# dhruvmetha/rapid-locomotion-rl

Hardware: AMD Instinct MI355X
Metric: env-steps/sec, 4096 Mini Cheetah envs, 1/2/4/8 MI355X; PPO iters/sec (higher is better)
Workload: dtype f32; 1 GPU; 4096 Mini Cheetah envs flat terrain (4096 per GPU), PPO teacher policy (BASELINE configs[1]); envs_per_gpu=4096, global_envs=4096, global_batch_env_steps_per_iter=98304, parallelism=dp1, world_size=1, policy=ActorCritic 42/18/630->12, random init; teacher PPO + student adaptation update

## Files before the change

### include/lrl.h

```cpp
#ifndef LRL_H_
#define LRL_H_

#include <stddef.h>
#include <stdint.h>

#ifdef __cplusplus
extern "C" {
#endif

#define LRL_ABI_VERSION 6

#define LRL_OK 0
#define LRL_E_INVALID (-1)
#define LRL_E_HIP (-2)
#define LRL_E_NOMEM (-3)
#define LRL_E_NOGPU (-4)

#define LRL_MAX_BODIES 20
#define LRL_MAX_SPHERES 40
#define LRL_NUM_DOF 12
#define LRL_NUM_LEGS 4
#define LRL_MAX_OBS 256
#define LRL_MAX_HEIGHT_POINTS 192
#define LRL_MAX_REWARD_TERMS 24
// ... 516 lines not shown
                           int32_t zero, void* stream);

int32_t lrl_curriculum_sample(uint32_t* mt_key, int32_t* mt_pos, const double* weights, int32_t nbins,
                              const double* grid, const double* half, int32_t n, double* cmds, int64_t* bins);
int32_t lrl_curriculum_update_weights(double* weights, const double* axes, int32_t nx, int32_t ny, int32_t nz,
                                      const int64_t* centres, int32_t n, double local_range);
double lrl_np_sum_f64(const double* a, int64_t n);

#ifdef __cplusplus
}
#endif

#include "lrl_vision.h"
#include "lrl_depth_sense.h"
#include "lrl_history_shift.h"

#endif
```

### rapid-locomotion-rl_amd/csrc/lrl_ppo.hip

```cpp
#include <hip/hip_runtime.h>
#include <math.h>
#include <stdint.h>
#include <stdlib.h>
#include <string.h>

#include <algorithm>
#include <initializer_list>
#include <mutex>
#include <vector>

#include "../../include/lrl.h"
#include "../../include/lrl_philox.h"
#include "lrl_gemm.h"
#include "lrl_launch.h"

namespace lrl {

constexpr float LOG_SQRT_2PI = 0.91893853320467274178f;
constexpr int HEAD_ROWS = 32;
constexpr int HEAD_THREADS = 256;
constexpr int HEAD_W = 128;
constexpr int MAX_ACT = 16;
constexpr int HEAD_NA = 12;
constexpr int MAX_LAT = 32;
// ... 272 lines not shown
    }
    P[hp_b4a(NA) + t] = sb;
    P[hp_std(NA) + t] = ss;
  } else if (t == 16) {
    float sb = 0.f;
    for (int r = 0; r < nrows; ++r) sb += DR[r][1];
    P[hp_b4c(NA)] = sb;
  } else if (t >= 32 && t < 35) {
    const int c = t - 32;
    float s = 0.f;
    for (int r = 0; r < nrows; ++r) s += SC[r][c];
    P[hp_kl(NA) + c] = s;
  }
}

struct ActHeadArgs {
  const float* h3;
  const float *w4a, *b4a, *w4c, *b4c, *stdv;
  const float *obs, *priv, *hist, *eps;
  int n, na, no, np;
  uint64_t seed, counter;
  int64_t row_offset;
  float *actions, *mu, *values, *logp;
  lrl_rollout_store store;
  int store_row, do_store;
  float* xa_out;
  float* hist_shift;
  int hist_slot;
};

template <int NT = HEAD_THREADS>
__device__ __forceinline__ void copy_rows(const float* __restrict__ src, int64_t sld, float* __restrict__ dst,
                                          int64_t dld, int nrows, int cols, int t) {
  if (((((uintptr_t)src | (uintptr_t)dst) & 7) == 0) && (((sld | dld | cols) & 1) == 0)) {
    const int c2 = cols / 2, n = nrows * c2;
    for (int i0 = t; i0 < n; i0 += 8 * NT) {
      float2 v[8];
#pragma unroll
      for (int u = 0; u < 8; ++u) {
        const int i = i0 + u * NT, r = i / c2, c = i - r * c2;
        if (i < n) v[u] = reinterpret_cast<const float2*>(src + r * sld)[c];
      }
#pragma unroll
// ... 131 lines not shown
    const float m = MU[r][j], sd = a.stdv[j];
    float act;
    MU[r][j] = act_draw(a.eps, a.row_offset, a.seed, a.counter, g, j, na, m, sd, act);
    a.actions[(int64_t)g * na + j] = act;
    if (a.mu) a.mu[(int64_t)g * na + j] = m;
    if (a.do_store) {
      const int64_t o = (so + g) * na + j;
      a.store.actions[o] = act;
      a.store.mu[o] = m;
      a.store.sigma[o] = sd;
    }
  }
  __syncthreads();
  if (t < nrows) {
    const int g = r0 + t;
    float lp = 0.f;
    for (int j = 0; j < na; ++j) lp += MU[t][j];
    float vs[ACT_Q];
#pragma unroll
    for (int q = 0; q < ACT_Q; ++q) vs[q] = VP[t][q];
#pragma unroll
    for (int w = ACT_Q / 2; w >= 1; w /= 2)
#pragma unroll
      for (int q = 0; q < w; ++q) vs[q] = vs[2 * q] + vs[2 * q + 1];
    const float v = vs[0] + a.b4c[0];
    if (a.values) a.values[g] = v;
    if (a.logp) a.logp[g] = lp;
    if (a.do_store) {
      a.store.values[so + g] = v;
      a.store.logp[so + g] = lp;
// ... 167 lines not shown

struct FusedActArgs {
  const float* w;
  lrl_ppo_net net;
  const float *obs, *priv, *hist, *eps;
  int n, xs;
  uint32_t vec;
  uint64_t seed, counter;
  int64_t row_offset;
  float *actions, *mu, *values, *logp;
  lrl_rollout_store store;
  int store_row, do_store;
  float* xa_out;
  float* hist_shift;
  int hist_slot;
};

template <bool PRESET, int RB>
__device__ __forceinline__ void fa_encoder(const FusedActArgs& a, float* X, float* HE1, float* MID, int r0, int nrows,
                                           unsigned long long& fa_t) {
  constexpr int R = 16 * RB, NT = 256 * RB;
  const lrl_ppo_net& nt = a.net;
  const int t = threadIdx.x;
  const int no = nt.num_obs, np = nt.num_priv, PP = 36, EP2 = nt.enc_h1 + 4;
  for (int e = t; e < R * a.xs; e += NT) {
    const int r = e / a.xs, c = e - r * a.xs;
    X[r * FA_XP + c] = (r < nrows && c < no) ? a.obs[(int64_t)(r0 + r) * no + c] : 0.f;
  }
  for (int e = t; e < R * 32; e += NT) {
    const int r = e >> 5, c = e & 31;
// ... 247 lines not shown
          const int64_t o = (so + g) * NA + j;
          a.store.actions[o] = act;
          a.store.mu[o] = m;
          a.store.sigma[o] = sd;
        }
      }
      __syncthreads();
      if (t < nrows) {
        const int g = r0 + t;
        float lp = 0.f;
        for (int j = 0; j < NA; ++j) lp += MU[t * 16 + j];
        if (a.logp) a.logp[g] = lp;
        if (a.do_store) a.store.logp[so + g] = lp;
      }
    } else {
      for (int e = t; e < HEAD_W; e += OA_THREADS) HW[e] = w[nt.w4c + e];
      __syncthreads();
      for (int e = t; e < OA_R * 16; e += OA_THREADS) {
        const int r = e & (OA_R - 1), q = e / OA_R;
        float s = 0.f;
        for (int k = q * (HEAD_W / 16); k < (q + 1) * (HEAD_W / 16); ++k) s = fmaf(H3[r * OA_H3P + k], HW[k], s);
        VP[r * 16 + q] = s;
      }
      __syncthreads();
      FA_PROF(8)
      if (t < nrows) {
        const int g = r0 + t;
        float vs[16];
#pragma unroll
        for (int q = 0; q < 16; ++q) vs[q] = VP[t * 16 + q];
// ... 740 lines not shown
  if (reset) {
    unsigned long long z[12] = {0};
    if (hipMemcpyToSymbol(HIP_SYMBOL(g_act_prof), z, sizeof(z)) != hipSuccess) return -2;
  }
  return 12;
#else
  (void)out;
  (void)reset;
  return 0;
#endif
}

static int32_t ppo_act(const lrl_ppo_net* net, const float* params, const float* obs, const float* priv,
                       const float* hist, int32_t n, const float* eps, uint64_t seed, uint64_t counter,
                       int64_t row_offset, float* actions, float* mu, float* values, float* logp, const lrl_rollout_store* store,
                       int32_t store_row, void* workspace, void* stream, float* hist_shift, int32_t hist_slot) {
  if (int rc = check_net(net)) return rc;
  if (hist_shift && (hist_shift != hist || !store || !store->hist || hist_slot <= 0 || store->hist_dim % hist_slot != 0))
    return lrl_set_error(LRL_E_INVALID, "lrl_ppo_act_shift: hist_shift must be hist, with a history store and a slot "
                                        "width that divides its hist_dim");
  if (!params || !obs || (!priv && !net->plain) || !actions || !workspace || n <= 0)
    return lrl_set_error(LRL_E_INVALID, "lrl_ppo_act: null argument or n <= 0");
  if (store && (!store->obs || (!store->priv && priv) || !store->actions || !store->values || !store->logp ||
                !store->mu || !store->sigma || store->hist_dim < 0 ||
                (store->hist_ld != 0 && store->hist_ld < store->hist_dim)))
    return lrl_set_error(LRL_E_INVALID, "lrl_ppo_act: incomplete rollout store");
  const lrl_ppo_net& nt = *net;
  hipStream_t st = static_cast<hipStream_t>(stream);
  auto io = [&](auto& a) {
    a.obs = obs; a.priv = priv; a.hist = hist; a.eps = eps; a.n = n;
    a.seed = seed; a.counter = counter; a.row_offset = row_offset;
    a.actions = actions; a.mu = mu; a.values = values; a.logp = logp;
    if (store) a.store = *store;
    a.store_row = store_row; a.do_store = store ? 1 : 0;
    a.hist_shift = hist_shift; a.hist_slot = hist_slot;
  };
  const bool full = !nt.plain;
  if (full && fused_act_fits(nt, n)) {
    static const bool ok = [] {
      auto set = [](const void* f) {
        return hipFuncSetAttribute(f, hipFuncAttributeMaxDynamicSharedMemorySize, OA_LDS_BYTES) == hipSuccess;
      };
      return set(reinterpret_cast<const void*>(act_fused_kernel<true>)) &&
             set(reinterpret_cast<const void*>(act_fused_kernel<false>));
    }();
    if (!ok) return lrl_set_error(LRL_E_HIP, "lrl_ppo_act: fused kernel LDS attribute");
    FusedActArgs fa{};
    fa.w = params; fa.net = nt; fa.xs = xs_of(nt);
    io(fa);
    launch_act_fused(fa, true, st);
// ... 30 lines not shown
extern "C" int32_t lrl_ppo_act(const lrl_ppo_net* net, const float* params, const float* obs, const float* priv,
                               const float* hist, int32_t n, const float* eps, uint64_t seed, uint64_t counter,
                               int64_t row_offset, float* actions, float* mu, float* values, float* logp, const lrl_rollout_store* store,
                               int32_t store_row, void* workspace, void* stream) {
  return ppo_act(net, params, obs, priv, hist, n, eps, seed, counter, row_offset, actions, mu, values, logp, store, store_row,
                 workspace, stream, nullptr, 0);
}

extern "C" int32_t lrl_ppo_act_shift(const lrl_ppo_net* net, const float* params, const float* obs, const float* priv,
                                     const float* hist, int32_t n, const float* eps, uint64_t seed, uint64_t counter,
                                     int64_t row_offset, float* actions, float* mu, float* values, float* logp,
                                     const lrl_rollout_store* store, int32_t store_row, void* workspace, void* stream,
                                     float* hist_shift, int32_t hist_slot) {
  return ppo_act(net, params, obs, priv, hist, n, eps, seed, counter, row_offset, actions, mu, values, logp, store, store_row,
                 workspace, stream, hist_shift, hist_slot);
}

extern "C" int64_t lrl_ppo_act_student_workspace_bytes(const lrl_ppo_net* net, int32_t n) {
  if (check_net(net) || net->plain || n <= 0) return -1;
  return make_student_plan(*net, n, nullptr).bytes;
}

extern "C" int32_t lrl_ppo_act_student(const lrl_ppo_net* net, const float* params, const float* obs,
                                       const float* hist, int32_t hist_ld, int32_t n, float* mean, float* latent,
                                       void* workspace, void* stream) {
  if (int rc = check_net(net)) return rc;
  if (net->plain) return lrl_set_error(LRL_E_INVALID, "lrl_ppo_act_student: a plain net has no adaptation module");
  if (!params || !obs || !hist || !mean || !workspace || n <= 0)
    return lrl_set_error(LRL_E_INVALID, "lrl_ppo_act_student: null argument or n <= 0");
  const lrl_ppo_net& nt = *net;
// ... 11 lines not shown
  body_forward(g, L.body, P);
  g.forward(L.mean, P.h3, nullptr, Buf{mean, nt.num_actions}, false);
  if (g.rc) return lrl_set_error(g.rc, "lrl_ppo_act_student: GEMM launch failed");
  if (latent &&
      hipMemcpy2DAsync(latent, (size_t)nt.latent * 4, lat.p, (size_t)lat.ld * 4, (size_t)nt.latent * 4, n,
                       hipMemcpyDeviceToDevice, st) != hipSuccess)
    return lrl_set_error(LRL_E_HIP, "lrl_ppo_act_student: latent copy failed");
  return hipGetLastError() == hipSuccess ? 0 : lrl_set_error(LRL_E_HIP, "lrl_ppo_act_student: launch failed");
}

extern "C" int64_t lrl_ppo_workspace_bytes(const lrl_ppo_net* net, int32_t batch) {
  if (check_net(net) || batch <= 0) return -1;
  return make_plan(*net, batch, nullptr).bytes;
}

extern "C" int32_t lrl_ppo_forward_backward(const lrl_ppo_net* net, const float* params, float* grads,
                                            const lrl_ppo_batch* bt, const lrl_ppo_hparams* hp, void* workspace,
                                            lrl_ppo_ctrl* ctrl, void* stream) {
  if (int rc = check_net(net)) return rc;
  if (!bt || !hp || !params || !grads || !workspace || !ctrl || bt->batch <= 0)
    return lrl_set_error(LRL_E_INVALID, "lrl_ppo_forward_backward: null argument");
  const lrl_ppo_net& n = *net;
  const int B = bt->batch;
  const bool full = !n.plain;
  Plan P = make_plan(n, B, static_cast<char*>(workspace));
  hipStream_t st = static_cast<hipStream_t>(stream);
  G g{st, params, B, P.part, P.part + P.part_floats};
  g.tanh_act = n.plain;
  const Net net_l = layers_of(n);
  const Layer(&enc)[3] = net_l.enc;
  const Layer(&body)[3] = net_l.body;
  PlaneJob pj[PL_MAIN];
  if (full) {
    main_plane_jobs(n, params, P.wpl, pj);
    if (int rc = split_planes(pj, PL_MAIN, gemm_x6p_enabled(), st))
      return lrl_set_error(rc, "lrl_ppo_forward_backward: planes launch failed");
    g.with(pj);
  }
  const In priv{bt->priv, n.num_priv};
  prep_x(n, bt->obs, bt->rows, B, P.xa, st);
  if (full) encoder_forward(g, enc, priv, bt->rows, P, cols_from(P.xa, n.num_obs));
  body_forward(g, body, P);
  if (g.rc) return lrl_set_error(g.rc, "lrl_ppo_forward_backward: forward GEMM launch failed");
  SegList L{};
  launch_loss_head(n, params, grads, bt, hp, ctrl, P, g.part, L, st);
  g.backward_data(body[2], P.dh3, P.dh2, P.h2);
  g.backward_data(body[1], P.dh2, P.dh1, P.h1);
  if (full) g.backward_data(net_l.dlat, P.dh1, P.dlat, In{});
  enum { DWE3, DHE2, DWE2, DHE1, DWE1, DW3, DW2, DW1, NJOBS };
  GemmJob jobs[NJOBS];
  const int first = full ? 0 : DW3;
  g.collect(jobs, first, NJOBS);
  if (full) {
    g.weight_grad(enc[2], P.dlat, P.he2, nullptr, grads, L);
    g.backward_data(enc[2], P.dlat, P.dhe2, P.he2);
// ... 29 lines not shown
    return lrl_set_error(LRL_E_HIP, "lrl_ppo_forward_backward: stream fork failed");
  for (int s = 0; s < ns && !rc; ++s) {
    const int lead = sets[s].i[0];
    const bool timed = full && sets[s].n == 1 && lead == DW2;
    if (timed) timer_begin(st);
    rc = launch_jobs(jobs, sets[s].i, sets[s].n, fk && lead < DW3 ? fk->st : st);
    if (timed) timer_end(st);
    if (fk && lead == DWE1 && hipEventRecord(fk->done, fk->st) != hipSuccess)
      return lrl_set_error(LRL_E_HIP, "lrl_ppo_forward_backward: stream fork failed");
  }
  if (fk && hipStreamWaitEvent(st, fk->done, 0) != hipSuccess)
    return lrl_set_error(LRL_E_HIP, "lrl_ppo_forward_backward: stream join failed");
  if (rc) return lrl_set_error(rc, "lrl_ppo_forward_backward: backward GEMM launch failed");
  launch_seg(L, st);
  return hipGetLastError() == hipSuccess ? 0 : lrl_set_error(LRL_E_HIP, "lrl_ppo_forward_backward: launch failed");
}

extern "C" int32_t lrl_ppo_optimizer_step(const lrl_ppo_net* net, float* params, const float* grads, float* exp_avg,
                                          float* exp_avg_sq, int64_t step, float grad_scale,
                                          const lrl_ppo_hparams* hp, void* workspace, lrl_ppo_ctrl* ctrl,
                                          void* stream) {
  if (int rc = check_net(net)) return rc;
  if (!params || !grads || !exp_avg || !exp_avg_sq || !hp || !workspace || !ctrl || step < 1)
    return lrl_set_error(LRL_E_INVALID, "lrl_ppo_optimizer_step: bad argument");
  const lrl_ppo_net& n = *net;
  hipStream_t st = static_cast<hipStream_t>(stream);
  double* norm_part = static_cast<double*>(workspace);
  const int64_t len = n.main_end - n.main_begin;
  hipLaunchKernelGGL(sumsq_kernel, dim3(NORM_BLOCKS), dim3(256), 0, st, grads + n.main_begin, len, norm_part);
  const double bc1 = 1.0 - pow((double)hp->beta1, (double)step);
// ... 248 lines not shown
```

### rapid-locomotion-rl_amd/lrl/_abi.py

```python
import ctypes as C
import os
import re

_HERE = os.path.dirname(os.path.abspath(__file__))
LIB_PATH = os.environ.get("LRL_LIB") or os.path.join(os.path.dirname(_HERE), "csrc", "liblrl.so")

MAX_BODIES, MAX_SPHERES, NUM_DOF, NUM_LEGS, MAX_OBS, MAX_REWARD_TERMS, NUM_PRIV = 20, 40, 12, 4, 256, 24, 18
MAX_HEIGHT_POINTS = 192
f32, i32, u32 = C.c_float, C.c_int32, C.c_uint32

REWARD_TERMS = ["lin_vel_z", "ang_vel_xy", "orientation", "base_height", "torques", "energy",
                "energy_expenditure", "dof_vel", "dof_acc", "action_rate", "collision", "survival",
                "dof_pos_limits", "dof_vel_limits", "torque_limits", "tracking_lin_vel", "tracking_ang_vel",
                "feet_air_time", "stumble", "stand_still", "feet_contact_forces"]

STEP_PHYSICS, STEP_HISTORY, STEP_INJECT_UNIFORM = 1, 2, 4

(T_ROOT_STATE, T_DOF_POS, T_DOF_VEL, T_CONTACT_FORCE, T_RIGID_BODY_STATE, T_TORQUES, T_ACTIONS, T_LAST_ACTIONS,
 T_LAST_DOF_VEL, T_LAST_ROOT_VEL, T_COMMANDS, T_OBS, T_PRIV_OBS, T_OBS_HISTORY, T_REWARD, T_RESET, T_TIME_OUT,
 T_EPISODE_LENGTH, T_EPISODE_SUMS, T_COMMAND_SUMS, T_FEET_AIR_TIME, T_LAST_CONTACTS, T_FRICTION, T_RESTITUTION,
 T_PAYLOAD, T_COM_DISPLACEMENT, T_MOTOR_STRENGTH, T_KP_FACTOR, T_KD_FACTOR, T_ENV_ORIGINS, T_BASE_LIN_VEL,
 T_BASE_ANG_VEL, T_PROJECTED_GRAVITY, T_JOINT_POS_TARGET, T_MEASURED_HEIGHTS, T_NUM) = range(36)


# ... 194 lines not shown
    return struct


def _fill_array(arr, v):
    for i, x in enumerate(v):
        if isinstance(arr[i], C.Array):
            _fill_array(arr[i], x)
        else:
            arr[i] = x


_CSRC = os.path.join(os.path.dirname(_HERE), "csrc")
_HEADER = os.path.join(os.path.dirname(os.path.dirname(_HERE)), "include", "lrl.h")
_SENSE_HEADER = os.path.join(os.path.dirname(_HEADER), "lrl_depth_sense.h")
_SHIFT_HEADER = os.path.join(os.path.dirname(_HEADER), "lrl_history_shift.h")


def source_hash():
    import hashlib
    with open(os.path.join(_CSRC, "Makefile")) as f:
        mk = f.read()
    h = hashlib.sha256()
    for var in ("SRCS", "HDRS"):
        for name in re.search(rf"^{var} = (.*)$", mk, re.M).group(1).split():
            with open(os.path.join(_CSRC, name), "rb") as f:
                h.update(f.read())
    return h.hexdigest()[:16]


MIRRORS = {"lrl_model": LrlModel, "lrl_env_params": LrlEnvParams, "lrl_group_params": LrlGroupParams,
# ... 36 lines not shown

_lib = None


def lib():
    global _lib
    if _lib is None:
        if not os.path.exists(LIB_PATH):
            raise RuntimeError(f"liblrl.so not built ({LIB_PATH}); run __graft_entry__.build()")
        L = C.CDLL(LIB_PATH)
        L.lrl_build_hash.restype = C.c_char_p
        built, want = L.lrl_build_hash().decode(), source_hash()
        if built != want and not os.environ.get("LRL_LIB"):
            raise RuntimeError(f"{LIB_PATH} was built from other sources (hash {built}, tree {want}); "
                               "rebuild it: __graft_entry__.build()")
        for header in (_HEADER, _SENSE_HEADER, _SHIFT_HEADER):
            with open(header) as f:
                for name, (restype, argtypes) in signatures(f.read()).items():
                    fn = getattr(L, name)
                    fn.restype, fn.argtypes = restype, argtypes
        _lib = L
    return _lib


def check(rc):
    if rc != 0:
        msg = lib().lrl_last_error()
        raise RuntimeError(f"liblrl error {rc}: {msg.decode() if msg else ''}")
    return rc


# ... 13 lines not shown
```

### rapid-locomotion-rl_amd/lrl/ppo/actor_critic.py

```python
import ctypes as C

import torch

import torch.nn as nn

from .. import _abi
from ..config import ArgsProto


class AC_Args(ArgsProto):
    init_noise_std = 1.0
    actor_hidden_dims = [512, 256, 128]
    critic_hidden_dims = [512, 256, 128]
    activation = "elu"
    adaptation_module_branch_hidden_dims = [[256, 32]]
    env_factor_encoder_branch_input_dims = [18]
    env_factor_encoder_branch_latent_dims = [18]
    env_factor_encoder_branch_hidden_dims = [[256, 128]]


def get_activation(name):
    return {"elu": nn.ELU(), "selu": nn.SELU(), "relu": nn.ReLU(), "crelu": nn.ReLU(), "lrelu": nn.LeakyReLU(),
            "tanh": nn.Tanh(), "sigmoid": nn.Sigmoid()}.get(name)

# ... 147 lines not shown
        net = self.flatten_parameters()
        ws = getattr(self, "_student_ws", None)
        if ws is None or ws[0] != n or ws[1].device != dev:
            nbytes = _abi.lib().lrl_ppo_act_student_workspace_bytes(C.byref(net), n)
            if nbytes < 0:
                raise RuntimeError("lrl_ppo_act_student_workspace_bytes rejected the network")
            ws = self._student_ws = (n, torch.empty(nbytes, dtype=torch.uint8, device=dev))
        mean = torch.empty(n, self.num_actions, device=dev)
        latent = torch.empty(n, net.latent, device=dev)
        _abi.check(_abi.lib().lrl_ppo_act_student(net, self._flat.data_ptr(), obs.data_ptr(), hist.data_ptr(),
                                                  hist.stride(0), n, mean.data_ptr(), latent.data_ptr(),
                                                  ws[1].data_ptr(), _abi.stream_of(dev)))
        return mean, latent

    def act_fused(self, obs, priv, hist=None, eps=None, seed=0, counter=0, store=None, store_row=0, row_offset=0,
                  shift_history=False):
        n = obs.shape[0]
        dev = obs.device
        assert obs.is_contiguous() and (priv is None or priv.is_contiguous()) and obs.dtype == torch.float32
        net = self.flatten_parameters()
        ws = getattr(self, "_act_ws", None)
        if ws is None or ws[0] != n or ws[1].device != dev:
            nbytes = _abi.lib().lrl_ppo_act_workspace_bytes(C.byref(net), n)
            if nbytes < 0:
                raise RuntimeError("lrl_ppo_act_workspace_bytes rejected the network")
            ws = self._act_ws = (n, torch.empty(nbytes, dtype=torch.uint8, device=dev))
        actions = torch.empty(n, self.num_actions, device=dev)
        mu = torch.empty(n, self.num_actions, device=dev)
        values = torch.empty(n, 1, device=dev)
        logp = torch.empty(n, device=dev)
        priv_p, hist_p, eps_p = (t.data_ptr() if t is not None else None for t in (priv, hist, eps))
        if shift_history:
            if hist is None or store is None or not hist.is_contiguous():
                raise ValueError("shift_history needs a contiguous history and a rollout store")
            _abi.check(_abi.lib().lrl_ppo_act_shift(net, self._flat.data_ptr(), obs.data_ptr(), priv_p, hist_p, n, eps_p,
                                                    seed, counter, row_offset, actions.data_ptr(), mu.data_ptr(),
                                                    values.data_ptr(), logp.data_ptr(), store, store_row,
                                                    ws[1].data_ptr(), _abi.stream_of(dev), hist_p, obs.shape[1]))
            return actions, mu, values, logp
        _abi.check(_abi.lib().lrl_ppo_act(net, self._flat.data_ptr(), obs.data_ptr(), priv_p, hist_p, n, eps_p, seed,
                                          counter, row_offset, actions.data_ptr(), mu.data_ptr(), values.data_ptr(),
                                          logp.data_ptr(), store, store_row, ws[1].data_ptr(), _abi.stream_of(dev)))
        return actions, mu, values, logp
```

### rapid-locomotion-rl_amd/lrl/ppo/ppo.py

```python
import ctypes as C
import os

import torch

import torch.distributed as dist
import torch.nn as nn
import torch.nn.functional as F

from .. import _abi
from ..config import ArgsProto
from .actor_critic import ActorCritic
from .rollout_storage import RolloutStorage


_SNAPSHOTS = max(2, int(os.environ.get("LRL_ENC_SNAPSHOTS", "4")))


class PPO_Args(ArgsProto):
    value_loss_coef = 1.0
    use_clipped_value_loss = True
    clip_param = 0.2
    entropy_coef = 0.01
    num_learning_epochs = 5
    num_mini_batches = 4
# ... 41 lines not shown
                                                            lr=self.args.adaptation_module_learning_rate)
        self.transition = RolloutStorage.Transition()
        self._lr = float(self.args.learning_rate)
        self.async_losses = False
        self._lr_dev = None
        self.fused = (torch.device(device).type == "cuda") if fused is None else fused
        self.seed = seed
        self.row_offset = 0
        self._act_counter = 0
        self._store = None
        self.grad_allreduce = _collective()
        self._native = None
        self.record_lr = False
        self.overlap_adaptation = True
        self.lr_trace = []
        if self.fused:
            self.actor_critic.flatten_parameters()

    def init_storage(self, num_envs, num_transitions_per_env, actor_obs_shape, privileged_obs_shape, obs_history_shape,
                     action_shape):
        self.storage = self.storage_class(num_envs, num_transitions_per_env, actor_obs_shape, privileged_obs_shape,
                                          obs_history_shape, action_shape, self.device)
        self._store = self.storage.store_desc() if self.fused else None

    def test_mode(self):
        self.actor_critic.eval()

    def train_mode(self):
        self.actor_critic.train()

    def act(self, obs, privileged_obs, obs_history, eps=None, shift_history=False):
        if shift_history and not (self.fused and obs_history.is_contiguous()):
            raise ValueError("shift_history needs the native act and a contiguous history")
        if self.fused:
            self._act_counter += 1
            a, mu, v, lp = self.actor_critic.act_fused(
                obs.contiguous(), privileged_obs.contiguous(), obs_history.contiguous(), eps=eps, seed=self.seed,
                counter=self._act_counter, store=self._store, store_row=self.storage.step,
                row_offset=self.row_offset, shift_history=shift_history)
            t = self.transition
            t.actions, t.values, t.actions_log_prob, t.action_mean = a, v, lp, mu
            t.action_sigma = self.actor_critic.std.detach().expand_as(mu)
            t.observations = t.critic_observations = obs
            t.privileged_observations, t.observation_histories = privileged_obs, obs_history
            return a
        t = self.transition
        t.actions = self.actor_critic.act(obs, privileged_obs).detach()
        t.values = self.actor_critic.evaluate(obs, privileged_obs).detach()
        t.actions_log_prob = self.actor_critic.get_actions_log_prob(t.actions).detach()
        t.action_mean = self.actor_critic.action_mean.detach()
        t.action_sigma = self.actor_critic.action_std.detach()
        t.observations = t.critic_observations = obs
        t.privileged_observations, t.observation_histories = privileged_obs, obs_history
        return t.actions
# ... 12 lines not shown
        self.storage.add_transitions(t, fused=self.fused)
        t.clear()
        self.actor_critic.reset(dones)

    def _store_step(self, rewards, dones, infos):
        s, t = self.storage, self.transition
        bins, tout = infos["env_bins"], infos.get("time_outs")
        n = s.num_envs
        ok = lambda x, dt: (x.dtype == dt and x.is_cuda and x.is_contiguous() and x.numel() == n)
        if not (ok(rewards, torch.float32) and ok(dones, torch.bool) and ok(bins, torch.float32)):
            return False
        if tout is not None and not (ok(tout, torch.bool) and ok(t.values, torch.float32)):
            return False
        if s.step >= s.num_transitions_per_env:
            raise AssertionError("Rollout buffer overflow")
        i = s.step
        values, tout = (t.values.data_ptr(), tout.data_ptr()) if tout is not None else (None, None)
        _abi.check(_abi.lib().lrl_ppo_store_step(rewards.data_ptr(), dones.data_ptr(), bins.data_ptr(), values, tout,
                                                 float(self.args.gamma), n, s.rewards[i].data_ptr(),
                                                 s.dones[i].data_ptr(), s.env_bins[i].data_ptr(),
                                                 _abi.stream_of(rewards.device)))
        s.step += 1
        return True

    def compute_returns(self, last_critic_obs, last_critic_privileged_obs):
        if self.fused:
            _, _, last_values, _ = self.actor_critic.act_fused(last_critic_obs.contiguous(),
                                                               last_critic_privileged_obs.contiguous(),
                                                               seed=self.seed, counter=0, row_offset=self.row_offset)
        else:
            last_values = self.actor_critic.evaluate(last_critic_obs, last_critic_privileged_obs).detach()
        reduce = None
        if _collective():
            reduce = _all_reduce_
        self.storage.compute_returns(last_values, self.args.gamma, self.args.lam, reduce_stats=reduce)

    def _allreduce_grads(self, params):
        grads = [p.grad for p in params if p.grad is not None]
        if not grads:
            return
        flat = torch.cat([g.reshape(-1) for g in grads])
        _all_reduce_(flat)
        flat /= _world()
        off = 0
        for g in grads:
# ... 15 lines not shown
            _abi.fill(hp, clip_param=self.args.clip_param, entropy_coef=self.args.entropy_coef,
                      value_loss_coef=self.args.value_loss_coef, max_grad_norm=self.args.max_grad_norm,
                      desired_kl=self.args.desired_kl if self.args.desired_kl is not None else 0.0,
                      use_clipped_value_loss=int(self.args.use_clipped_value_loss),
                      adaptive_schedule=int(self.args.desired_kl is not None and self.args.schedule == "adaptive"),
                      beta1=0.9, beta2=0.999, eps=1e-8)
            st["hp"] = hp
            self._native = st
        if st["ws_batch"] != batch:
            nbytes = _abi.lib().lrl_ppo_workspace_bytes(C.byref(net), batch)
            if nbytes < 0:
                raise RuntimeError("lrl_ppo_workspace_bytes rejected the network")
            st["ws"] = torch.empty(nbytes, dtype=torch.uint8, device=ac._flat.device)
            st["ws_b"] = st["ws"] if net.plain else torch.empty(nbytes, dtype=torch.uint8, device=ac._flat.device)
            st["ws_batch"] = batch
        return st

    @property
    def learning_rate(self):
        if self._lr_dev is not None:
            self._lr = float(self._lr_dev[0].item())
            self._lr_dev = None
            for g in self.optimizer.param_groups:
                g["lr"] = self._lr
        return self._lr

    @learning_rate.setter
    def learning_rate(self, v):
        self._lr = float(v)
        self._lr_dev = None

    def _update_native(self, sync=True):
        s = self.storage
        T, N = s.num_transitions_per_env, s.num_envs
        nmb = self.args.num_mini_batches
        mb = (T * N) // nmb
        st = self._native_state(mb)
        net, hp = st["net"], st["hp"]
        world = _world()
        coll = _collective()
        L = _abi.lib()
        stream = _abi.stream_of(st["grads"].device)
        indices = torch.randperm(nmb * mb, requires_grad=False, device=self.device)
        trace = []
        flat = lambda t: t.flatten(0, 1)
        bufs = dict(obs=flat(s.observations), priv=flat(s.privileged_observations),
                    hist=flat(s.observation_histories), actions=flat(s.actions), values=flat(s.values),
# ... 21 lines not shown
                sb = st["stream_b"] = torch.cuda.Stream(params.device)
            stream_b, ws_b = sb.cuda_stream, st["ws_b"]
            if "enc_snap" not in st:
                st["enc_snap"] = [torch.zeros(net.total, device=params.device) for _ in range(_SNAPSHOTS)]
            e0, e1 = net.e1w, net.std_off
        else:
            sb, stream_b, ws_b = cur, stream, ws
        params_p, grads_p, m_p, v_p, ws_p, ws_b_p, ctrl_p = (t.data_ptr()
                                                             for t in (params, grads, m, v, ws, ws_b, ctrl))
        adapt_lr = float(self.args.adaptation_module_learning_rate)
        batch_b = _abi.LrlPpoBatch()
        C.memmove(C.byref(batch_b), C.byref(batch), C.sizeof(batch))
        if sb is not cur and "read_done_ev" not in st:
            st["read_done_ev"] = [torch.cuda.Event() for _ in range(_SNAPSHOTS)]
        read_done = [None] * _SNAPSHOTS
        k = 0
        for epoch in range(self.args.num_learning_epochs):
            for i in range(nmb):
                rows = indices[i * mb:(i + 1) * mb]
                batch.rows = rows.data_ptr()
                _abi.check(L.lrl_ppo_forward_backward(net, params_p, grads_p, batch, hp, ws_p, ctrl_p, stream))
                if coll:
                    _all_reduce_(main)
                st["steps"][0] += 1
                _abi.check(L.lrl_ppo_optimizer_step(net, params_p, grads_p, m_p, v_p, st["steps"][0], scale, hp, ws_p,
                                                    ctrl_p, stream))
                if self.record_lr:
                    trace.append(ctrl[0].clone())
                enc = None
                if sb is not cur:
                    snap = st["enc_snap"][k % _SNAPSHOTS]
                    if read_done[k % _SNAPSHOTS] is not None:
                        cur.wait_event(read_done[k % _SNAPSHOTS])
                    snap[e0:e1].copy_(params[e0:e1])
                    enc = snap.data_ptr()
                    sb.wait_stream(cur)
# ... 109 lines not shown
```

### rapid-locomotion-rl_amd/lrl/ppo/rollout_storage.py

```python

import torch

from .. import _abi


class RolloutStorage:
    class Transition:
        def __init__(self):
            self.observations = None
            self.privileged_observations = None
            self.observation_histories = None
            self.critic_observations = None
            self.actions = None
            self.rewards = None
            self.dones = None
            self.values = None
            self.actions_log_prob = None
            self.action_mean = None
            self.action_sigma = None
            self.env_bins = None

        def clear(self):
            self.__init__()

# ... 15 lines not shown
            self.observation_histories = z(*obs_history_shape)
        self.rewards = z(1)
        self.actions = z(*actions_shape)
        self.dones = z(1).byte()
        self.actions_log_prob = z(1)
        self.values = z(1)
        self.returns = z(1)
        self.advantages = z(1)
        self.mu = z(*actions_shape)
        self.sigma = z(*actions_shape)
        self.env_bins = z(1)
        self.num_transitions_per_env, self.num_envs = T, N
        self.step = 0
        self._ws = None
        self.adv_stats = None

    def store_desc(self):
        s = _abi.LrlRolloutStore()
        s.obs, s.priv, s.hist = (self.observations.data_ptr(), self.privileged_observations.data_ptr(),
                                 self.observation_histories.data_ptr())
        s.actions, s.values, s.logp = self.actions.data_ptr(), self.values.data_ptr(), self.actions_log_prob.data_ptr()
        s.mu, s.sigma = self.mu.data_ptr(), self.sigma.data_ptr()
        s.hist_dim = self.obs_history_shape[0]
        s.hist_ld = self.observation_histories.stride(1)
        return s

    def add_transitions(self, transition, fused=False):
        if self.step >= self.num_transitions_per_env:
            raise AssertionError("Rollout buffer overflow")
        t = self.step
# ... 4 lines not shown
            self.actions[t].copy_(transition.actions)
            self.values[t].copy_(transition.values)
            self.actions_log_prob[t].copy_(transition.actions_log_prob.view(-1, 1))
            self.mu[t].copy_(transition.action_mean)
            self.sigma[t].copy_(transition.action_sigma)
        self.rewards[t].copy_(transition.rewards.view(-1, 1))
        self.dones[t].copy_(transition.dones.view(-1, 1))
        self.env_bins[t].copy_(transition.env_bins.view(-1, 1))
        self.step += 1

    def clear(self):
        self.step = 0

    def compute_returns(self, last_values, gamma, lam, reduce_stats=None):
        T, N = self.num_transitions_per_env, self.num_envs
        if self._ws is None:
            self._ws = torch.empty(4096, device=self.device)
        lv = last_values.contiguous().float()
        stream = _abi.stream_of(self.rewards.device)
        args = (self.rewards.data_ptr(), self.dones.data_ptr(), self.values.data_ptr(), lv.data_ptr(), T, N,
                float(gamma), float(lam), self.returns.data_ptr(), self.advantages.data_ptr(), self._ws.data_ptr())
        if reduce_stats is None:
            _abi.check(_abi.lib().lrl_gae(*args, stream))
        else:
            stats = torch.empty(3, dtype=torch.float64, device=self.device)
            _abi.check(_abi.lib().lrl_gae_partial(*args, stats.data_ptr(), stream))
            stats = reduce_stats(stats)
            _abi.check(_abi.lib().lrl_adv_normalize(self.advantages.data_ptr(), T * N, stats.data_ptr(), stream))

    def mini_batch_generator(self, num_mini_batches, num_epochs=8):
        batch_size = self.num_envs * self.num_transitions_per_env
        mb = batch_size // num_mini_batches
        indices = torch.randperm(num_mini_batches * mb, requires_grad=False, device=self.device)
        flat = lambda t: t.flatten(0, 1)
        obs, priv, hist = flat(self.observations), flat(self.privileged_observations), flat(self.observation_histories)
        actions, values, returns = flat(self.actions), flat(self.values), flat(self.returns)
        logp, adv, mu, sigma, bins = (flat(self.actions_log_prob), flat(self.advantages), flat(self.mu),
                                      flat(self.sigma), flat(self.env_bins))
        for epoch in range(num_epochs):
            for i in range(num_mini_batches):
                idx = indices[i * mb:(i + 1) * mb]
                yield (obs[idx], obs[idx], priv[idx], hist[idx], actions[idx], values[idx], adv[idx], returns[idx],
                       logp[idx], mu[idx], sigma[idx], None, bins[idx])
```

### rapid-locomotion-rl_amd/lrl/ppo/runner.py

```python
import copy
import os

import torch

from ml_logger import ML_Logger, logger as _ml_logger

from ..config import ArgsProto
from .actor_critic import ActorCritic
from .ppo import PPO


_SYNC_UPDATE = os.environ.get("LRL_RUNNER_SYNC", "0") == "1"


class RunnerArgs(ArgsProto):
    algorithm_class_name = "PPO"
    num_steps_per_env = 24
    max_iterations = 1500
    save_interval = 400
    save_video_interval = 100
    log_freq = 10
    resume = False
    load_run = -1
    checkpoint = -1
# ... 32 lines not shown
        self.logger = logger if logger is not None else _ml_logger
        self.env.reset()
        self.eval_metrics = None
        if getattr(self.args, "log_eval_metrics", False) and getattr(self.env, "num_eval_envs", 0) > 0:
            from ..eval_metrics import EvalMetrics
            self.eval_metrics = EvalMetrics(self.env).enable()

    def learn(self, num_learning_iterations, init_at_random_ep_len=False, eval_freq=100, eval_expert=False):
        lg = self.logger
        lg.start("start", "epoch", "episode", "run", "step")
        if init_at_random_ep_len:
            self.env.episode_length_buf = torch.randint_like(self.env.episode_length_buf,
                                                             high=int(self.env.max_episode_length))
        n_train = self.env.num_train_envs
        shift_ok = os.environ.get("LRL_ACT_SHIFT_HISTORY", "1") != "0"
        obs_dict = self.env.get_observations()
        obs, priv, hist = obs_dict["obs"], obs_dict["privileged_obs"], obs_dict["obs_history"]
        self.alg.actor_critic.train()
        tot_iter = self.current_learning_iteration + num_learning_iterations
        for it in range(self.current_learning_iteration, tot_iter):
            with torch.inference_mode():
                for _ in range(self.num_steps_per_env):
                    shift = shift_ok and self.alg.fused and self._is_env_history(hist, n_train)
                    actions = self.alg.act(obs[:n_train], priv[:n_train], hist[:n_train], shift_history=shift)
                    if shift:
                        self.env.history_preshifted(n_train)
                    if self.env.num_envs > n_train:
                        actions = torch.cat((actions, self._eval_actions(obs, priv, hist, n_train, eval_expert)), 0)
                    obs_dict, rewards, dones, infos = self.env.step(actions)
                    obs, priv, hist = obs_dict["obs"], obs_dict["privileged_obs"], obs_dict["obs_history"]
# ... 8 lines not shown
                        with lg.Prefix(metrics="eval/metrics"):
                            lg.store_metrics(self.eval_metrics.summary("eval"))
                        self.eval_metrics.clear()
                    self.env.reset_evaluation_envs()
            mv, ms, ma = self.alg.update()
            lg.store_metrics(time_elapsed=lg.since("start"), time_iter=lg.split("epoch"), adaptation_loss=ma,
                             mean_value_loss=mv, mean_surrogate_loss=ms)
            if self.args.save_video_interval:
                self.log_video(it)
            self.tot_timesteps += self.num_steps_per_env * self.env.num_envs
            if lg.every(self.args.log_freq, "iteration", start_on=1):
                lg.log_metrics_summary(key_values={"timesteps": self.tot_timesteps, "iterations": it})
                lg.job_running()
            if self.args.save_interval and it % self.args.save_interval == 0:
                self.save(it)
        self.current_learning_iteration += num_learning_iterations
        if num_learning_iterations > 0:
            self.save(tot_iter - 1)

    def _is_env_history(self, hist, n_train):
        buf = getattr(self.env, "obs_history_buf", None)
        return (isinstance(buf, torch.Tensor) and hasattr(self.env, "history_preshifted") and hist.is_contiguous()
                and buf.is_contiguous() and hist.data_ptr() == buf.data_ptr() and hist.shape == buf.shape
                and hist.dtype == torch.float32 and 0 < n_train <= buf.shape[0])

    def log_video(self, it):
        env = self.env
        if not hasattr(env, "start_recording") or not hasattr(env, "camera_props"):
            return
        lg = self.logger
# ... 48 lines not shown
```

Measured before the change: 4.208 million env-steps/s.

## Fuse rollout store-step into act kernel and cache PPO input buffers across epochs

```diff
diff --git a/include/lrl.h b/include/lrl.h
--- a/include/lrl.h
+++ b/include/lrl.h
@@ -554,5 +554,6 @@
 #include "lrl_vision.h"
 #include "lrl_depth_sense.h"
 #include "lrl_history_shift.h"
+#include "lrl_ppo_critpath.h"
 
 #endif
diff --git a/include/lrl_ppo_critpath.h b/include/lrl_ppo_critpath.h
--- /dev/null
+++ b/include/lrl_ppo_critpath.h
@@ -0,0 +1,28 @@
+#ifndef LRL_PPO_CRITPATH_H_
+#define LRL_PPO_CRITPATH_H_
+
+#include <stdint.h>
+
+#ifdef __cplusplus
+extern "C" {
+#endif
+
+int64_t lrl_ppo_x_floats(const lrl_ppo_net* net, int32_t batch);
+
+int32_t lrl_ppo_forward_backward_x(const lrl_ppo_net* net, const float* params, float* grads,
+                                   const lrl_ppo_batch* batch, const lrl_ppo_hparams* hp, void* workspace,
+                                   lrl_ppo_ctrl* ctrl, void* stream, float* x, int32_t x_ready);
+
+int32_t lrl_ppo_act_store_step(const lrl_ppo_net* net, const float* params, const float* obs, const float* priv,
+                               const float* hist, int32_t n, const float* eps, uint64_t seed, uint64_t counter,
+                               int64_t row_offset, float* actions, float* mu, float* values, float* logp,
+                               const lrl_rollout_store* store, int32_t store_row, void* workspace, void* stream,
+                               float* hist_shift, int32_t hist_slot, const float* rew, const uint8_t* done,
+                               const float* env_bins, const float* prev_values, const uint8_t* time_outs, float gamma,
+                               float* dst_rew, uint8_t* dst_done, float* dst_env_bins);
+
+#ifdef __cplusplus
+}
+#endif
+
+#endif
diff --git a/rapid-locomotion-rl_amd/csrc/lrl_ppo.hip b/rapid-locomotion-rl_amd/csrc/lrl_ppo.hip
--- a/rapid-locomotion-rl_amd/csrc/lrl_ppo.hip
+++ b/rapid-locomotion-rl_amd/csrc/lrl_ppo.hip
@@ -310,6 +310,29 @@
   }
 }
 
+struct StoreStepArgs {
+  const float* rew;
+  const uint8_t* done;
+  const float *bins, *values;
+  const uint8_t* time_outs;
+  float gamma;
+  float* dst_rew;
+  uint8_t* dst_done;
+  float* dst_bins;
+};
+__device__ __forceinline__ void store_step_row(const StoreStepArgs& s, int i) {
+#pragma clang fp contract(off)
+  float r = s.rew[i];
+  if (s.time_outs) {
+    const float vt = s.values[i] * (s.time_outs[i] ? 1.f : 0.f);
+    const float b = s.gamma * vt;
+    r = r + b;
+  }
+  s.dst_rew[i] = r;
+  s.dst_done[i] = s.done[i] ? 1 : 0;
+  if (s.bins) s.dst_bins[i] = s.bins[i];
+}
+
 struct ActHeadArgs {
   const float* h3;
   const float *w4a, *b4a, *w4c, *b4c, *stdv;
@@ -323,6 +346,7 @@
   float* xa_out;
   float* hist_shift;
   int hist_slot;
+  StoreStepArgs ss;
 };
 
 template <int NT = HEAD_THREADS>
@@ -484,6 +508,7 @@
   __syncthreads();
   if (t < nrows) {
     const int g = r0 + t;
+    if (a.ss.rew) store_step_row(a.ss, g);
     float lp = 0.f;
     for (int j = 0; j < na; ++j) lp += MU[t][j];
     float vs[ACT_Q];
@@ -681,6 +706,7 @@
   float* xa_out;
   float* hist_shift;
   int hist_slot;
+  StoreStepArgs ss;
 };
 
 template <bool PRESET, int RB>
@@ -958,6 +984,7 @@
         if (a.do_store) a.store.logp[so + g] = lp;
       }
     } else {
+      if (a.ss.rew && t < nrows) store_step_row(a.ss, r0 + t);
       for (int e = t; e < HEAD_W; e += OA_THREADS) HW[e] = w[nt.w4c + e];
       __syncthreads();
       for (int e = t; e < OA_R * 16; e += OA_THREADS) {
@@ -1728,7 +1755,8 @@
 static int32_t ppo_act(const lrl_ppo_net* net, const float* params, const float* obs, const float* priv,
                        const float* hist, int32_t n, const float* eps, uint64_t seed, uint64_t counter,
                        int64_t row_offset, float* actions, float* mu, float* values, float* logp, const lrl_rollout_store* store,
-                       int32_t store_row, void* workspace, void* stream, float* hist_shift, int32_t hist_slot) {
+                       int32_t store_row, void* workspace, void* stream, float* hist_shift, int32_t hist_slot,
+                       const StoreStepArgs* ss = nullptr) {
   if (int rc = check_net(net)) return rc;
   if (hist_shift && (hist_shift != hist || !store || !store->hist || hist_slot <= 0 || store->hist_dim % hist_slot != 0))
     return lrl_set_error(LRL_E_INVALID, "lrl_ppo_act_shift: hist_shift must be hist, with a history store and a slot "
@@ -1748,6 +1776,7 @@
     if (store) a.store = *store;
     a.store_row = store_row; a.do_store = store ? 1 : 0;
     a.hist_shift = hist_shift; a.hist_slot = hist_slot;
+    a.ss = ss ? *ss : StoreStepArgs{};
   };
   const bool full = !nt.plain;
   if (full && fused_act_fits(nt, n)) {
@@ -1808,6 +1837,24 @@
                                      float* hist_shift, int32_t hist_slot) {
   return ppo_act(net, params, obs, priv, hist, n, eps, seed, counter, row_offset, actions, mu, values, logp, store, store_row,
                  workspace, stream, hist_shift, hist_slot);
+}
+
+extern "C" int32_t lrl_ppo_act_store_step(const lrl_ppo_net* net, const float* params, const float* obs,
+                                          const float* priv, const float* hist, int32_t n, const float* eps,
+                                          uint64_t seed, uint64_t counter, int64_t row_offset, float* actions, float* mu,
+                                          float* values, float* logp, const lrl_rollout_store* store, int32_t store_row,
+                                          void* workspace, void* stream, float* hist_shift, int32_t hist_slot,
+                                          const float* rew, const uint8_t* done, const float* env_bins,
+                                          const float* prev_values, const uint8_t* time_outs, float gamma,
+                                          float* dst_rew, uint8_t* dst_done, float* dst_env_bins) {
+  if (!rew)
+    return ppo_act(net, params, obs, priv, hist, n, eps, seed, counter, row_offset, actions, mu, values, logp, store,
+                   store_row, workspace, stream, hist_shift, hist_slot);
+  if (!done || !dst_rew || !dst_done || (env_bins && !dst_env_bins) || (time_outs && !prev_values))
+    return lrl_set_error(LRL_E_INVALID, "lrl_ppo_act_store_step: incomplete store-step arguments");
+  const StoreStepArgs ss{rew, done, env_bins, prev_values, time_outs, gamma, dst_rew, dst_done, dst_env_bins};
+  return ppo_act(net, params, obs, priv, hist, n, eps, seed, counter, row_offset, actions, mu, values, logp, store,
+                 store_row, workspace, stream, hist_shift, hist_slot, &ss);
 }
 
 extern "C" int64_t lrl_ppo_act_student_workspace_bytes(const lrl_ppo_net* net, int32_t n) {
@@ -1849,9 +1896,9 @@
   return make_plan(*net, batch, nullptr).bytes;
 }
 
-extern "C" int32_t lrl_ppo_forward_backward(const lrl_ppo_net* net, const float* params, float* grads,
-                                            const lrl_ppo_batch* bt, const lrl_ppo_hparams* hp, void* workspace,
-                                            lrl_ppo_ctrl* ctrl, void* stream) {
+static int32_t ppo_forward_backward(const lrl_ppo_net* net, const float* params, float* grads, const lrl_ppo_batch* bt,
+                                    const lrl_ppo_hparams* hp, void* workspace, lrl_ppo_ctrl* ctrl, void* stream,
+                                    float* x, bool x_ready) {
   if (int rc = check_net(net)) return rc;
   if (!bt || !hp || !params || !grads || !workspace || !ctrl || bt->batch <= 0)
     return lrl_set_error(LRL_E_INVALID, "lrl_ppo_forward_backward: null argument");
@@ -1859,6 +1906,7 @@
   const int B = bt->batch;
   const bool full = !n.plain;
   Plan P = make_plan(n, B, static_cast<char*>(workspace));
+  if (x) P.xa.p = x;
   hipStream_t st = static_cast<hipStream_t>(stream);
   G g{st, params, B, P.part, P.part + P.part_floats};
   g.tanh_act = n.plain;
@@ -1873,7 +1921,7 @@
     g.with(pj);
   }
   const In priv{bt->priv, n.num_priv};
-  prep_x(n, bt->obs, bt->rows, B, P.xa, st);
+  if (!(x && x_ready)) prep_x(n, bt->obs, bt->rows, B, P.xa, st);
   if (full) encoder_forward(g, enc, priv, bt->rows, P, cols_from(P.xa, n.num_obs));
   body_forward(g, body, P);
   if (g.rc) return lrl_set_error(g.rc, "lrl_ppo_forward_backward: forward GEMM launch failed");
@@ -1933,6 +1981,26 @@
   if (rc) return lrl_set_error(rc, "lrl_ppo_forward_backward: backward GEMM launch failed");
   launch_seg(L, st);
   return hipGetLastError() == hipSuccess ? 0 : lrl_set_error(LRL_E_HIP, "lrl_ppo_forward_backward: launch failed");
+}
+
+extern "C" int32_t lrl_ppo_forward_backward(const lrl_ppo_net* net, const float* params, float* grads,
+                                            const lrl_ppo_batch* bt, const lrl_ppo_hparams* hp, void* workspace,
+                                            lrl_ppo_ctrl* ctrl, void* stream) {
+  return ppo_forward_backward(net, params, grads, bt, hp, workspace, ctrl, stream, nullptr, false);
+}
+
+extern "C" int64_t lrl_ppo_x_floats(const lrl_ppo_net* net, int32_t batch) {
+  if (check_net(net) || batch <= 0) return -1;
+  return (int64_t)batch * xs_of(*net);
+}
+
+extern "C" int32_t lrl_ppo_forward_backward_x(const lrl_ppo_net* net, const float* params, float* grads,
+                                              const lrl_ppo_batch* bt, const lrl_ppo_hparams* hp, void* workspace,
+                                              lrl_ppo_ctrl* ctrl, void* stream, float* x, int32_t x_ready) {
+  if (!x && x_ready) return lrl_set_error(LRL_E_INVALID, "lrl_ppo_forward_backward_x: x_ready without an X buffer");
+  const char* e = getenv("LRL_X_CACHE");
+  if (e && e[0] == '0') x = nullptr, x_ready = 0;
+  return ppo_forward_backward(net, params, grads, bt, hp, workspace, ctrl, stream, x, x_ready != 0);
 }
 
 extern "C" int32_t lrl_ppo_optimizer_step(const lrl_ppo_net* net, float* params, const float* grads, float* exp_avg,
diff --git a/rapid-locomotion-rl_amd/lrl/_abi.py b/rapid-locomotion-rl_amd/lrl/_abi.py
--- a/rapid-locomotion-rl_amd/lrl/_abi.py
+++ b/rapid-locomotion-rl_amd/lrl/_abi.py
@@ -232,6 +232,7 @@
 _HEADER = os.path.join(os.path.dirname(os.path.dirname(_HERE)), "include", "lrl.h")
 _SENSE_HEADER = os.path.join(os.path.dirname(_HEADER), "lrl_depth_sense.h")
 _SHIFT_HEADER = os.path.join(os.path.dirname(_HEADER), "lrl_history_shift.h")
+_CRITPATH_HEADER = os.path.join(os.path.dirname(_HEADER), "lrl_ppo_critpath.h")
 
 
 def source_hash():
@@ -298,7 +299,7 @@
         if built != want and not os.environ.get("LRL_LIB"):
             raise RuntimeError(f"{LIB_PATH} was built from other sources (hash {built}, tree {want}); "
                                "rebuild it: __graft_entry__.build()")
-        for header in (_HEADER, _SENSE_HEADER, _SHIFT_HEADER):
+        for header in (_HEADER, _SENSE_HEADER, _SHIFT_HEADER, _CRITPATH_HEADER):
             with open(header) as f:
                 for name, (restype, argtypes) in signatures(f.read()).items():
                     fn = getattr(L, name)
diff --git a/rapid-locomotion-rl_amd/lrl/ppo/actor_critic.py b/rapid-locomotion-rl_amd/lrl/ppo/actor_critic.py
--- a/rapid-locomotion-rl_amd/lrl/ppo/actor_critic.py
+++ b/rapid-locomotion-rl_amd/lrl/ppo/actor_critic.py
@@ -185,7 +185,7 @@
         return mean, latent
 
     def act_fused(self, obs, priv, hist=None, eps=None, seed=0, counter=0, store=None, store_row=0, row_offset=0,
-                  shift_history=False):
+                  shift_history=False, store_step=None):
         n = obs.shape[0]
         dev = obs.device
         assert obs.is_contiguous() and (priv is None or priv.is_contiguous()) and obs.dtype == torch.float32
@@ -201,9 +201,17 @@
         values = torch.empty(n, 1, device=dev)
         logp = torch.empty(n, device=dev)
         priv_p, hist_p, eps_p = (t.data_ptr() if t is not None else None for t in (priv, hist, eps))
+        if shift_history and (hist is None or store is None or not hist.is_contiguous()):
+            raise ValueError("shift_history needs a contiguous history and a rollout store")
+        if store_step is not None:
+            shift = (hist_p, obs.shape[1]) if shift_history else (None, 0)
+            _abi.check(_abi.lib().lrl_ppo_act_store_step(net, self._flat.data_ptr(), obs.data_ptr(), priv_p, hist_p, n,
+                                                         eps_p, seed, counter, row_offset, actions.data_ptr(),
+                                                         mu.data_ptr(), values.data_ptr(), logp.data_ptr(), store,
+                                                         store_row, ws[1].data_ptr(), _abi.stream_of(dev), *shift,
+                                                         *store_step))
+            return actions, mu, values, logp
         if shift_history:
-            if hist is None or store is None or not hist.is_contiguous():
-                raise ValueError("shift_history needs a contiguous history and a rollout store")
             _abi.check(_abi.lib().lrl_ppo_act_shift(net, self._flat.data_ptr(), obs.data_ptr(), priv_p, hist_p, n, eps_p,
                                                     seed, counter, row_offset, actions.data_ptr(), mu.data_ptr(),
                                                     values.data_ptr(), logp.data_ptr(), store, store_row,
diff --git a/rapid-locomotion-rl_amd/lrl/ppo/ppo.py b/rapid-locomotion-rl_amd/lrl/ppo/ppo.py
--- a/rapid-locomotion-rl_amd/lrl/ppo/ppo.py
+++ b/rapid-locomotion-rl_amd/lrl/ppo/ppo.py
@@ -79,6 +79,8 @@
         self.record_lr = False
         self.overlap_adaptation = True
         self.lr_trace = []
+        self.defer_store = False
+        self._pending = None
         if self.fused:
             self.actor_critic.flatten_parameters()
 
@@ -87,6 +89,7 @@
         self.storage = self.storage_class(num_envs, num_transitions_per_env, actor_obs_shape, privileged_obs_shape,
                                           obs_history_shape, action_shape, self.device)
         self._store = self.storage.store_desc() if self.fused else None
+        self.storage.before_read = self.flush_store
 
     def test_mode(self):
         self.actor_critic.eval()
@@ -102,7 +105,7 @@
             a, mu, v, lp = self.actor_critic.act_fused(
                 obs.contiguous(), privileged_obs.contiguous(), obs_history.contiguous(), eps=eps, seed=self.seed,
                 counter=self._act_counter, store=self._store, store_row=self.storage.step,
-                row_offset=self.row_offset, shift_history=shift_history)
+                row_offset=self.row_offset, shift_history=shift_history, store_step=self._take_store(obs.shape[0]))
             t = self.transition
             t.actions, t.values, t.actions_log_prob, t.action_mean = a, v, lp, mu
             t.action_sigma = self.actor_critic.std.detach().expand_as(mu)
@@ -145,21 +148,39 @@
             return False
         if s.step >= s.num_transitions_per_env:
             raise AssertionError("Rollout buffer overflow")
+        assert self._pending is None, "the env stepped again before an act (or flush_store) took the deferred store"
         i = s.step
+        keep = (rewards, dones, bins, t.values, tout)
         values, tout = (t.values.data_ptr(), tout.data_ptr()) if tout is not None else (None, None)
-        _abi.check(_abi.lib().lrl_ppo_store_step(rewards.data_ptr(), dones.data_ptr(), bins.data_ptr(), values, tout,
-                                                 float(self.args.gamma), n, s.rewards[i].data_ptr(),
-                                                 s.dones[i].data_ptr(), s.env_bins[i].data_ptr(),
-                                                 _abi.stream_of(rewards.device)))
+        ptrs = (rewards.data_ptr(), dones.data_ptr(), bins.data_ptr(), values, tout, float(self.args.gamma),
+                s.rewards[i].data_ptr(), s.dones[i].data_ptr(), s.env_bins[i].data_ptr())
+        self._pending = (ptrs, n, rewards.device, keep)
+        if not self.defer_store:
+            self.flush_store()
         s.step += 1
         return True
+
+    def flush_store(self):
+        if self._pending is not None:
+            ptrs, n, device, _ = self._pending
+            self._pending = None
+            _abi.check(_abi.lib().lrl_ppo_store_step(*ptrs[:6], n, *ptrs[6:], _abi.stream_of(device)))
+
+    def _take_store(self, n):
+        if self._pending is not None and self._pending[1] == n:
+            ptrs, self._pending = self._pending[0], None
+            return ptrs
+        self.flush_store()
+        return None
 
     def compute_returns(self, last_critic_obs, last_critic_privileged_obs):
         if self.fused:
             _, _, last_values, _ = self.actor_critic.act_fused(last_critic_obs.contiguous(),
                                                                last_critic_privileged_obs.contiguous(),
-                                                               seed=self.seed, counter=0, row_offset=self.row_offset)
+                                                               seed=self.seed, counter=0, row_offset=self.row_offset,
+                                                               store_step=self._take_store(last_critic_obs.shape[0]))
         else:
+            self.flush_store()
             last_values = self.actor_critic.evaluate(last_critic_obs, last_critic_privileged_obs).detach()
         reduce = None
         if _collective():
@@ -205,6 +226,13 @@
             st["ws"] = torch.empty(nbytes, dtype=torch.uint8, device=ac._flat.device)
             st["ws_b"] = st["ws"] if net.plain else torch.empty(nbytes, dtype=torch.uint8, device=ac._flat.device)
             st["ws_batch"] = batch
+            st["x_bufs"] = []
+        nmb = self.args.num_mini_batches
+        if len(st["x_bufs"]) != nmb:
+            floats = _abi.lib().lrl_ppo_x_floats(C.byref(net), batch)
+            if floats < 0:
+                raise RuntimeError("lrl_ppo_x_floats rejected the network")
+            st["x_bufs"] = [torch.empty(floats, device=ac._flat.device) for _ in range(nmb)]
         return st
 
     @property
@@ -222,6 +250,7 @@
         self._lr_dev = None
 
     def _update_native(self, sync=True):
+        self.flush_store()
         s = self.storage
         T, N = s.num_transitions_per_env, s.num_envs
         nmb = self.args.num_mini_batches
@@ -273,12 +302,15 @@
         if sb is not cur and "read_done_ev" not in st:
             st["read_done_ev"] = [torch.cuda.Event() for _ in range(_SNAPSHOTS)]
         read_done = [None] * _SNAPSHOTS
+        x_p = [x.data_ptr() for x in st["x_bufs"]]
         k = 0
         for epoch in range(self.args.num_learning_epochs):
+            x_ready = int(epoch > 0)
             for i in range(nmb):
                 rows = indices[i * mb:(i + 1) * mb]
                 batch.rows = rows.data_ptr()
-                _abi.check(L.lrl_ppo_forward_backward(net, params_p, grads_p, batch, hp, ws_p, ctrl_p, stream))
+                _abi.check(L.lrl_ppo_forward_backward_x(net, params_p, grads_p, batch, hp, ws_p, ctrl_p, stream,
+                                                        x_p[i], x_ready))
                 if coll:
                     _all_reduce_(main)
                 st["steps"][0] += 1
diff --git a/rapid-locomotion-rl_amd/lrl/ppo/rollout_storage.py b/rapid-locomotion-rl_amd/lrl/ppo/rollout_storage.py
--- a/rapid-locomotion-rl_amd/lrl/ppo/rollout_storage.py
+++ b/rapid-locomotion-rl_amd/lrl/ppo/rollout_storage.py
@@ -53,6 +53,7 @@
         self.step = 0
         self._ws = None
         self.adv_stats = None
+        self.before_read = None
 
     def store_desc(self):
         s = _abi.LrlRolloutStore()
@@ -87,6 +88,8 @@
 
     def compute_returns(self, last_values, gamma, lam, reduce_stats=None):
         T, N = self.num_transitions_per_env, self.num_envs
+        if self.before_read is not None:
+            self.before_read()
         if self._ws is None:
             self._ws = torch.empty(4096, device=self.device)
         lv = last_values.contiguous().float()
@@ -102,6 +105,8 @@
             _abi.check(_abi.lib().lrl_adv_normalize(self.advantages.data_ptr(), T * N, stats.data_ptr(), stream))
 
     def mini_batch_generator(self, num_mini_batches, num_epochs=8):
+        if self.before_read is not None:
+            self.before_read()
         batch_size = self.num_envs * self.num_transitions_per_env
         mb = batch_size // num_mini_batches
         indices = torch.randperm(num_mini_batches * mb, requires_grad=False, device=self.device)
diff --git a/rapid-locomotion-rl_amd/lrl/ppo/runner.py b/rapid-locomotion-rl_amd/lrl/ppo/runner.py
--- a/rapid-locomotion-rl_amd/lrl/ppo/runner.py
+++ b/rapid-locomotion-rl_amd/lrl/ppo/runner.py
@@ -70,6 +70,7 @@
                                                              high=int(self.env.max_episode_length))
         n_train = self.env.num_train_envs
         shift_ok = os.environ.get("LRL_ACT_SHIFT_HISTORY", "1") != "0"
+        self.alg.defer_store = self.alg.fused and os.environ.get("LRL_ACT_STORE_STEP", "1") != "0"
         obs_dict = self.env.get_observations()
         obs, priv, hist = obs_dict["obs"], obs_dict["privileged_obs"], obs_dict["obs_history"]
         self.alg.actor_critic.train()
@@ -108,6 +109,8 @@
                 lg.job_running()
             if self.args.save_interval and it % self.args.save_interval == 0:
                 self.save(it)
+        self.alg.flush_store()
+        self.alg.defer_store = False
         self.current_learning_iteration += num_learning_iterations
         if num_learning_iterations > 0:
             self.save(tot_iter - 1)
```

Measured after the change: 4.233 million env-steps/s (median of 6 runs). No clear change (+0.6%).
